# tsnorri/vcf2multialign

Hardware: AMD Instinct MI355X
Metric: aligned A2M Gbases/sec (higher is better)
Workload: dtype u8

## Files before the change

### vcf2multialign_amd/csrc/kernels.hpp

```cpp
#pragma once

#include <hip/hip_runtime.h>
#include <stdint.h>

#ifdef V2M_CHECKED_BUILD
__device__ uint32_t v2m_lds_poison_seed;
#endif

namespace v2m {

typedef uint32_t u32;
typedef uint64_t u64;

constexpr int kWave = 64;
typedef u32 vec4u __attribute__((ext_vector_type(4)));
typedef vec4u vec4u_unaligned8 __attribute__((aligned(8)));

#ifdef V2M_CHECKED_BUILD
__device__ __forceinline__ u32 poison_hash(u32 seed, u32 wg, u32 i)
{
	u32 h = seed ^ (wg * 0x9E3779B1u) ^ (i * 0x85EBCA77u);
	h ^= h >> 15; h *= 0x2C1B3C6Du;
	h ^= h >> 12; h *= 0x297A2D39u;
	h ^= h >> 15;
// ... 1413 lines not shown
{
	splice_aligned_tiles<kNonTemporal, true, true>(tmpl, eff, eff_words_per_row, tt, patches, labels, out, row_pitch, n_rows, rows_per_group, n_groups,
		n_tiles, tile_run, 0, gap, 0u, 0u, st);
}


__device__ __forceinline__ u32 zero_bytes_mask(u32 x)
{
	return ~(((x & 0x7F7F7F7Fu) + 0x7F7F7F7Fu) | x | 0x7F7F7F7Fu);
}

__device__ __forceinline__ u32 wave_inclusive_scan_u32(u32 v)
{
	v += (u32) __builtin_amdgcn_update_dpp(0, (int) v, 0x111, 0xf, 0xf, false);
	v += (u32) __builtin_amdgcn_update_dpp(0, (int) v, 0x112, 0xf, 0xf, false);
	v += (u32) __builtin_amdgcn_update_dpp(0, (int) v, 0x114, 0xf, 0xf, false);
	v += (u32) __builtin_amdgcn_update_dpp(0, (int) v, 0x118, 0xf, 0xf, false);
	v += (u32) __builtin_amdgcn_update_dpp(0, (int) v, 0x142, 0xa, 0xf, false);
	v += (u32) __builtin_amdgcn_update_dpp(0, (int) v, 0x143, 0xc, 0xf, false);
	return v;
}

template <int kN>
__device__ __forceinline__ void wave_inclusive_scan_u32_lockstep(u32 (&v)[kN])
{
#define V2M_SCAN_ROUND(CTRL, ROWS) \
	_Pragma("unroll") for (int k = 0; k < kN; ++k) v[k] += (u32) __builtin_amdgcn_update_dpp(0, (int) v[k], CTRL, ROWS, 0xf, false);
	V2M_SCAN_ROUND(0x111, 0xf)
	V2M_SCAN_ROUND(0x112, 0xf)
	V2M_SCAN_ROUND(0x114, 0xf)
	V2M_SCAN_ROUND(0x118, 0xf)
	V2M_SCAN_ROUND(0x142, 0xa)
	V2M_SCAN_ROUND(0x143, 0xc)
#undef V2M_SCAN_ROUND
}

__device__ __forceinline__ u64 wave_shift_left_u64(u64 v)
{
	u32 const lo = (u32) __builtin_amdgcn_update_dpp(0, (int) (u32) v, 0x130, 0xf, 0xf, true);
	u32 const hi = (u32) __builtin_amdgcn_update_dpp(0, (int) (u32) (v >> 32), 0x130, 0xf, 0xf, true);
	return (u64) hi << 32 | lo;
}

__device__ __forceinline__ u32 count_nonzero_bytes(unsigned char const *tile, u32 lo, u32 hi)
{
	u32 n = 0;
	while (lo < hi && (lo & 3)) n += tile[lo++] != 0;
	for (; lo + 4 <= hi; lo += 4)
		n += 4 - __builtin_popcount(zero_bytes_mask(*(u32 const *) (tile + lo)));
	while (lo < hi) n += tile[lo++] != 0;
	return n;
}

constexpr int kCountRowsMax = 256;
constexpr int kCandDeltaLds = 1024;

template <bool kWindow, bool kSet = false>
__device__ __forceinline__ void count_unaligned_tiles(
	vec4u const *__restrict__ tmpl0, u64 const *__restrict__ eff, u64 eff_words_per_row,
	tile_tables tt, edge_patch const *__restrict__ patches, char const *__restrict__ labels,
	u32 *__restrict__ tile_counts , u32 n_tiles,
	u32 n_rows, u32 rows_per_group, u32 n_groups, u32 tile_run, u32 col_base, u32 col_end, set_tile_tables const st = set_tile_tables{})
{
	__shared__ vec4u lds[kTileChunks];
	__shared__ patch_cache pc;
	__shared__ int row_delta[kCountRowsMax];
	__shared__ int cand_delta[kCandDeltaLds];
	__shared__ u32 wave_sums[kSpliceThreads / 64];

	int const t = threadIdx.x;
	u32 tile, group;
	map_block(blockIdx.x, n_groups, n_tiles, tile_run, tile, group);
	u32 const row_begin = group * rows_per_group;
	u32 const row_end = (row_begin + rows_per_group < n_rows) ? row_begin + rows_per_group : n_rows;
	V2M_POISON_LDS(lds);
	V2M_POISON_LDS(pc);
	V2M_POISON_LDS(row_delta);
	V2M_POISON_LDS(cand_delta);
	V2M_POISON_LDS(wave_sums);

	u32 const n_chunks = kSet ? set_tile_chunks(st, tile) : (u32) kTileChunks;
	u32 mine = 0;
#pragma unroll
	for (int k = 0; k < kChunksPerThread; ++k) {
		if (kSet && (u32) (t + kSpliceThreads * k) >= n_chunks) continue;
		vec4u const v = tmpl0[(kSet ? (u64) (st.record_offset[tile] >> 4) : (u64) tile * kTileChunks) + t + kSpliceThreads * k];
		lds[t + kSpliceThreads * k] = v;
#pragma unroll
		for (int d = 0; d < 4; ++d)
			mine += 4 - __builtin_popcount(zero_bytes_mask(v[d]));
	}
#pragma unroll
	for (int d = 32; d >= 1; d >>= 1) mine += __shfl_down(mine, d, kWave);
	if ((t & 63) == 0) wave_sums[t >> 6] = mine;
	for (u32 r = t; r < (u32) kCountRowsMax; r += kSpliceThreads) row_delta[r] = 0;

	tile_job job;
	load_patch_cache<kWindow, kSet>(pc, job, tt, patches, labels, eff, eff_words_per_row, tile, row_begin, row_end - row_begin, t, col_base, col_end, st);
	__syncthreads();
	u32 tile_count = 0;
#pragma unroll
	for (int wv = 0; wv < kSpliceThreads / 64; ++wv) tile_count += wave_sums[wv];

	unsigned char const *const tile_bytes = (unsigned char const *) lds;
	auto patch_delta = [&](tile_patch const &tp) {
		u32 const label_end = tp.aln_begin + tp.label_len;
		int const label_in_tile = label_end > tp.from ? (int) ((label_end < tp.to ? label_end : tp.to) - tp.from) : 0;
		return label_in_tile - (int) count_nonzero_bytes(tile_bytes, tp.from - job.tile_base, tp.to - job.tile_base);
	};
	u32 const n_cand = job.n_cross + job.n_range;
	for (u32 i = t; i < n_cand && i < (u32) kCandDeltaLds; i += kSpliceThreads)
		cand_delta[i] = patch_delta(candidate_patch<kWindow>(pc, job, patches, i, candidate_edge(job, tt, i), candidate_in_lds(job, i)));
	__syncthreads();
	for (u32 sub = row_begin; sub < row_end; sub += kGroupRowsLds) {
		u32 const sub_end = sub + kGroupRowsLds < row_end ? sub + kGroupRowsLds : row_end;
		if (sub != row_begin) {
			asm volatile("s_waitcnt lgkmcnt(0)" ::: "memory");
			__syncthreads();
			load_eff_cache(pc, job, eff, eff_words_per_row, sub, sub_end - sub, t);
			__syncthreads();
		}
		u32 const sub_rows = sub_end - sub;
		u32 const nw = job.n_lds ? ((job.range_begin + job.n_lds - 1) >> 6) - job.w0 + 1 : 0;
		for (u32 idx = t; idx < sub_rows * nw; idx += kSpliceThreads) {
			u32 const r = idx / nw, w = idx % nw;
			u32 const first = (job.w0 + w) * 64u;
			u64 bits = pc.eff[r][w];
			if (first < job.range_begin) bits &= ~0ULL << (job.range_begin - first);
			u32 const cached_end = job.range_begin + job.n_lds;
			if (cached_end < first + 64u) bits &= (1ULL << (cached_end - first)) - 1;
			int delta = 0;
			for (; bits; bits &= bits - 1) {
				u32 const e = first + (u32) __builtin_ctzll(bits);
				u32 const i = job.n_cross + (e - job.range_begin);
				delta += i < (u32) kCandDeltaLds ? cand_delta[i] : patch_delta(candidate_patch<kWindow>(pc, job, patches, i, e, true));
			}
			if (delta) atomicAdd(&row_delta[sub - row_begin + r], delta);
		}
		u32 const n_other = n_cand - job.n_lds;
		for (u32 idx = t; idx < sub_rows * n_other; idx += kSpliceThreads) {
			u32 const r = idx / n_other, j = idx % n_other;
			u32 const i = j < job.n_cross ? j : j + job.n_lds;
			u32 const e = candidate_edge(job, tt, i);
			if (!((eff[(u64) (sub + r) * eff_words_per_row + (e >> 6)] >> (e & 63)) & 1)) continue;
			int const delta = i < (u32) kCandDeltaLds ? cand_delta[i] : patch_delta(candidate_patch<kWindow>(pc, job, patches, i, e, false));
			if (delta) atomicAdd(&row_delta[sub - row_begin + r], delta);
		}
	}
	__syncthreads();
	for (u32 r = t; r < row_end - row_begin; r += kSpliceThreads)
		tile_counts[(u64) (row_begin + r) * n_tiles + tile] = (u32) ((int) tile_count + row_delta[r]);
}

__global__ __launch_bounds__(kSpliceThreads) void count_unaligned_kernel(
	vec4u const *__restrict__ tmpl0, u64 const *__restrict__ eff, u64 eff_words_per_row,
	tile_tables tt, edge_patch const *__restrict__ patches, char const *__restrict__ labels,
	u32 *__restrict__ tile_counts , u32 n_tiles,
	u32 n_rows, u32 rows_per_group, u32 n_groups, u32 tile_run)
{
	count_unaligned_tiles<false>(tmpl0, eff, eff_words_per_row, tt, patches, labels, tile_counts, n_tiles, n_rows, rows_per_group, n_groups, tile_run, 0u, 0u);
}

__global__ __launch_bounds__(kSpliceThreads) void count_unaligned_window_kernel(
	vec4u const *__restrict__ tmpl0, u64 const *__restrict__ eff, u64 eff_words_per_row,
	tile_tables tt, edge_patch const *__restrict__ patches, char const *__restrict__ labels,
	u32 *__restrict__ tile_counts , u32 n_tiles,
	u32 n_rows, u32 rows_per_group, u32 n_groups, u32 tile_run, u32 col_base, u32 col_end)
{
	count_unaligned_tiles<true>(tmpl0, eff, eff_words_per_row, tt, patches, labels, tile_counts, n_tiles, n_rows, rows_per_group, n_groups, tile_run, col_base, col_end);
}

__global__ __launch_bounds__(kSpliceThreads) void count_unaligned_set_kernel(
	vec4u const *__restrict__ tmpl0, u64 const *__restrict__ eff, u64 eff_words_per_row,
	tile_tables tt, set_tile_tables st, edge_patch const *__restrict__ patches, char const *__restrict__ labels,
	u32 *__restrict__ tile_counts , u32 n_tiles,
	u32 n_rows, u32 rows_per_group, u32 n_groups, u32 tile_run)
{
	count_unaligned_tiles<true, true>(tmpl0, eff, eff_words_per_row, tt, patches, labels, tile_counts, n_tiles, n_rows, rows_per_group, n_groups, tile_run, 0u, 0u, st);
}

__device__ __forceinline__ u32 compaction_selector(u32 keep)
{
	u32 sel = 0x0c0c0c0cu, n = 0;
	for (u32 b = 0; b < 4; ++b)
		if (keep >> b & 1) { sel = (sel & ~(0xFFu << (8 * n))) | (b << (8 * n)); ++n; }
	return sel;
}

typedef unsigned short u16;
typedef u16 u16_unaligned __attribute__((aligned(1)));
typedef u32 u32_unaligned __attribute__((aligned(1)));
typedef u64 u64_unaligned __attribute__((aligned(1)));
typedef vec4u vec4u_unaligned __attribute__((aligned(1)));

#ifdef V2M_TUNING_BUILD
template <bool kNonTemporal>
__global__ __launch_bounds__(kSpliceThreads) void splice_unaligned_per_wave_kernel(
	vec4u const *__restrict__ tmpl0, u64 const *__restrict__ eff, u64 eff_words_per_row,
	tile_tables tt, edge_patch const *__restrict__ patches, char const *__restrict__ labels,
	u32 const *__restrict__ tile_offsets , u32 n_tiles,
	char *__restrict__ out, u64 row_pitch, u32 n_rows, u32 rows_per_group, u32 n_groups, u32 tile_run)
{
	__shared__ vec4u lds[kTileChunks];
	__shared__ patch_cache pc;
	__shared__ u32 wave_sums[kChunksPerThread * (kSpliceThreads / 64)];
	__shared__ u32 compact_sel[16];
	constexpr u32 kPackQueue = 24;
	__shared__ u32 pack_queue[kSpliceThreads / 64][kPackQueue];

	int const t = threadIdx.x;
	int const lane = t & 63, wave = __builtin_amdgcn_readfirstlane(t >> 6);
	if (t < 16) compact_sel[t] = compaction_selector((u32) t);
	u32 tile, group;
	map_block(blockIdx.x, n_groups, n_tiles, tile_run, tile, group);
	{
		u32 const t0 = tile / tile_run * tile_run;
		u32 const run = (n_tiles - t0 < tile_run) ? n_tiles - t0 : tile_run;
		if (0 == run % 8) { u32 const j = tile - t0; tile = t0 + (j & 7) * (run / 8) + (j >> 3); }
	}
	u32 const row_begin = group * rows_per_group;
	u32 const row_end = (row_begin + rows_per_group < n_rows) ? row_begin + rows_per_group : n_rows;

	vec4u pristine[kChunksPerThread];
#pragma unroll
	for (int k = 0; k < kChunksPerThread; ++k)
		pristine[k] = tmpl0[(u64) tile * kTileChunks + t + kSpliceThreads * k];

	tile_job job;
	load_patch_cache(pc, job, tt, patches, labels, eff, eff_words_per_row, tile, row_begin, row_end - row_begin, t);

	for (u32 row = row_begin; row < row_end; ++row) {
// ... 1115 lines not shown
```

### vcf2multialign_amd/csrc/v2m_hip.hip

```cpp

#include <hip/hip_runtime.h>

#include <algorithm>
#include <atomic>
#include <chrono>
#include <condition_variable>
#include <cstdarg>
#include <cstdio>
#include <cstdlib>
#include <cstring>
#include <functional>
#include <memory>
#include <mutex>
#include <string>
#include <thread>
#include <utility>
#include <vector>

#include <type_traits>
#include <unordered_map>

#include "../../include/v2m_hip.h"
#include "kernels.hpp"
#include "founder_kernels.hpp"
// ... 80 lines not shown
		hipError_t const st(dev_buf::ensure(n));
#ifdef V2M_CHECKED_BUILD
		if (hipSuccess == st && !fresh) return poison_device(p, bytes);
#else
		(void) fresh;
#endif
		return st;
	}
};

struct pinned_buf {
	void *p{};
	size_t bytes{};
	~pinned_buf() { reset(); }
	void reset() { if (p) (void) hipHostFree(p); p = nullptr; bytes = 0; }
	hipError_t ensure(size_t n)
	{
		if (n <= bytes) return hipSuccess;
		reset();
		if (0 == n) return hipSuccess;
		hipError_t const st(hipHostMalloc(&p, n, hipHostMallocDefault));
		if (hipSuccess == st) bytes = n; else p = nullptr;
		return st;
	}
	template <typename T> T *as() const { return static_cast<T *>(p); }
};

struct event_pair { hipEvent_t begin{}, end{}; };

}


struct held_ring_state {
	std::mutex mutex;
	std::condition_variable released;
};

struct v2m_row_hold {
	pinned_buf host;
	hipEvent_t copied{};
	uint64_t outstanding{};
	held_ring_state *ring{};
};


struct word_range { u64 restart, lo, hi, stride; };

struct row_view {
	u64 begin{}, end{};
	u64 max_unaligned{};
	u32 n_tiles{};
	dev_buf d_template, d_template0;
	bool has_template0{};
	dev_buf d_edge_begin, d_cross_offsets, d_cross_edges;
	word_range words{};
	u64 length() const { return end - begin; }
};


struct v2m_ctx {
	int device{};
	u32 n_cus{256};
	hipStream_t stream{};
	hipStream_t copy_stream{};
	std::string err;

	bool profiling{};
	std::vector<event_pair> events[V2M_KERNEL_LIMIT];
	std::vector<event_pair> free_events;

	bool has_graph{};
	u64 n_nodes{}, n_edges{}, ref_len{}, aligned_len{}, label_bytes{};
	bool has_nul_byte{};
	std::vector<u32> h_csum;
	std::vector<u32> h_tgt_prefix_max;
	dev_buf d_ref, d_ref_pos, d_aln_pos, d_spans, d_patches, d_labels, d_overlappable;
	dev_buf d_ovl_rank, d_blocker_masks;
	std::vector<u32> h_aln_pos, h_tile_edge_begin, h_cross_offsets, h_cross_edges;
	std::vector<v2m::edge_patch> h_patches;
	std::vector<u64> h_overlappable;

	row_view whole, window;
	bool windowed{};
	row_view &view() { return set_call ? set.view : windowed ? window : whole; }
	row_view const &view() const { return set_call ? set.view : windowed ? window : whole; }

	struct window_set {
		row_view view;
		u64 n_windows{}, pitch{}, mean_tile_bytes{};
		std::vector<u32> lengths;
		dev_buf d_col_begin, d_col_end, d_record_offset, d_edge_end, d_tile_window, d_first_tile, d_slot_offset32;
	} set;
	bool has_set{}, set_call{};
	scratch_buf d_set_tile_offsets, d_set_lengths[2];
	int set_lengths_slot{};
	scratch_buf d_distinct_keys, d_distinct_windows, d_distinct_items, d_distinct_flags;
	pinned_buf h_distinct_keys, h_distinct_items, h_distinct_flags;

	u64 const *d_paths{};
	dev_buf owned_paths;
	dev_buf d_slice_src;
	u64 path_rows{}, path_cols{};
	u64 path_pitch{};
	dev_buf d_by_edge;
	bool by_edge_valid{};

// ... 696 lines not shown
		launch(0 != mode);
	}
	V2M_HIP_TRY(ctx, hipGetLastError());
	return V2M_OK;
}


v2m::set_tile_tables set_tables(v2m_ctx const *ctx)
{
	auto const &s(ctx->set);
	return {s.d_col_begin.as<u32>(), s.d_col_end.as<u32>(), s.d_record_offset.as<u32>(), s.d_edge_end.as<u32>()};
}

int expand_reference_set(v2m_ctx *ctx, dev_buf &dst, char gap);


int splice_aligned_slice(v2m_ctx *ctx, v2m_row_batch const *rows, u64 row_begin, u64 row_end, char *d_out, u64 row_pitch)
{
	u64 const n_rows(row_end - row_begin);
	if (0 == n_rows || 0 == ctx->aligned_len) return V2M_OK;
	if (int const rc = resolve_slice(ctx, rows, row_begin, row_end)) return rc;

	row_view const &v(ctx->view());
	splice_grid g;
	if (int const rc = make_grid(ctx, n_rows, g)) return rc;
	v2m::tile_tables const tt{v.d_edge_begin.as<u32>(), v.d_cross_offsets.as<u32>(), v.d_cross_edges.as<u32>()};
	u64 const store_limit((v.length() + 15) & ~u64(15));
	auto const launch([&](bool nt) {
		auto const go([&](auto kernel, auto... window) {
			hipLaunchKernelGGL(kernel, dim3(unsigned(g.n_blocks)), dim3(v2m::kSpliceThreads), 0, ctx->stream,
				v.d_template.as<v2m::vec4u>(), ctx->d_eff.as<u64>() - v.words.restart, v.words.stride, tt, ctx->d_patches.as<v2m::edge_patch>(), ctx->d_labels.as<char>(),
				d_out, row_pitch, u32(n_rows), g.rows_per_group, g.n_groups, v.n_tiles, g.tile_run, store_limit, '-', window...);
		});
		if (ctx->set_call) {
			auto const go_set([&](auto kernel) {
				hipLaunchKernelGGL(kernel, dim3(unsigned(g.n_blocks)), dim3(v2m::kSpliceThreads), 0, ctx->stream,
					v.d_template.as<v2m::vec4u>(), ctx->d_eff.as<u64>() - v.words.restart, v.words.stride, tt, set_tables(ctx), ctx->d_patches.as<v2m::edge_patch>(), ctx->d_labels.as<char>(),
					d_out, row_pitch, u32(n_rows), g.rows_per_group, g.n_groups, v.n_tiles, g.tile_run, '-');
			});
			if (nt) go_set(v2m::splice_aligned_set_kernel<true>);
			else go_set(v2m::splice_aligned_set_kernel<false>);
		}
		else if (ctx->windowed) {
			if (nt) go(v2m::splice_aligned_window_kernel<true>, u32(v.begin), u32(v.end));
			else go(v2m::splice_aligned_window_kernel<false>, u32(v.begin), u32(v.end));
		}
		else if (nt) go(v2m::splice_aligned_kernel<true>);
		else go(v2m::splice_aligned_kernel<false>);
	});
	return store_flavour_launch(ctx, false, n_rows, n_rows * v.length(), launch);
}


int splice_unaligned_slice(v2m_ctx *ctx, v2m_row_batch const *rows, u64 row_begin, u64 row_end, char *d_out, u64 row_pitch)
{
	u64 const n_rows(row_end - row_begin);
	if (0 == n_rows) return V2M_OK;
	V2M_HIP_TRY(ctx, ctx->d_row_lengths.ensure(n_rows * sizeof(u64)));
	if (0 == ctx->aligned_len) {
		V2M_HIP_TRY(ctx, hipMemsetAsync(ctx->d_row_lengths.p, 0, n_rows * sizeof(u64), ctx->stream));
		return V2M_OK;
	}
	row_view &v(ctx->view());
	bool const set(ctx->set_call);
	if (!v.has_template0) {
		if (int const rc = set ? expand_reference_set(ctx, v.d_template0, 0) : expand_reference(ctx, v, v.d_template0, 0)) return rc;
		v.has_template0 = true;
	}
	if (int const rc = resolve_slice(ctx, rows, row_begin, row_end)) return rc;

	splice_grid g;
	if (int const rc = make_grid(ctx, n_rows, g)) return rc;
	V2M_HIP_TRY(ctx, ctx->d_tile_counts.ensure(n_rows * v.n_tiles * sizeof(u32)));
	if (set) {
		V2M_HIP_TRY(ctx, ctx->d_set_tile_offsets.ensure(n_rows * v.n_tiles * sizeof(u32)));
		V2M_HIP_TRY(ctx, ctx->d_set_lengths[ctx->set_lengths_slot].ensure(n_rows * ctx->set.n_windows * sizeof(u32)));
	}
	bool const windowed(ctx->windowed);
	v2m::tile_tables const tt{v.d_edge_begin.as<u32>(), v.d_cross_offsets.as<u32>(), v.d_cross_edges.as<u32>()};
	u64 const *const d_eff(ctx->d_eff.as<u64>() - v.words.restart);
	{
		char const *const ce(std::getenv("V2M_COUNT_ROWS_PER_GROUP"));
		u32 const count_rows(u32(std::min<u64>(std::max<u64>(1, n_rows), (ce && *ce && std::atoi(ce) > 0) ? u64(std::min(std::atoi(ce), int(v2m::kCountRowsMax))) : u64(v2m::kCountRowsMax))));
		u32 const count_groups(u32((n_rows + count_rows - 1) / count_rows));
		timed_launch tl(ctx, V2M_KERNEL_UNALIGNED_COUNT);
		auto const count([&](auto kernel, auto... window) {
			hipLaunchKernelGGL(kernel, dim3(unsigned(u64(v.n_tiles) * count_groups)), dim3(v2m::kSpliceThreads), 0, ctx->stream,
				v.d_template0.as<v2m::vec4u>(), d_eff, v.words.stride, tt, ctx->d_patches.as<v2m::edge_patch>(), ctx->d_labels.as<char>(),
				ctx->d_tile_counts.as<u32>(), v.n_tiles, u32(n_rows), count_rows, count_groups, g.tile_run, window...);
		});
		if (set)
			hipLaunchKernelGGL(v2m::count_unaligned_set_kernel, dim3(unsigned(u64(v.n_tiles) * count_groups)), dim3(v2m::kSpliceThreads), 0, ctx->stream,
				v.d_template0.as<v2m::vec4u>(), d_eff, v.words.stride, tt, set_tables(ctx), ctx->d_patches.as<v2m::edge_patch>(), ctx->d_labels.as<char>(),
				ctx->d_tile_counts.as<u32>(), v.n_tiles, u32(n_rows), count_rows, count_groups, g.tile_run);
		else if (windowed) count(v2m::count_unaligned_window_kernel, u32(v.begin), u32(v.end));
		else count(v2m::count_unaligned_kernel);
		hipLaunchKernelGGL(v2m::scan_tile_counts_kernel, dim3(unsigned(n_rows)), dim3(256), 0, ctx->stream,
			ctx->d_tile_counts.as<u32>(), v.n_tiles, ctx->d_row_lengths.as<u64>());
		if (set)
			hipLaunchKernelGGL(v2m::scan_window_set_kernel, dim3(unsigned(n_rows)), dim3(256), 0, ctx->stream,
				ctx->d_tile_counts.as<u32>(), ctx->d_row_lengths.as<u64>(), v.n_tiles, u32(ctx->set.n_windows),
				ctx->set.d_first_tile.as<u32>(), ctx->set.d_tile_window.as<u32>(), ctx->set.d_slot_offset32.as<u32>(),
				ctx->d_set_tile_offsets.as<u32>(), ctx->d_set_lengths[ctx->set_lengths_slot].as<u32>());
	}
	auto const launch([&](bool nt) {
		auto const go([&](auto kernel, auto... window) {
			hipLaunchKernelGGL(kernel, dim3(unsigned(g.n_blocks)), dim3(v2m::kSpliceThreads), 0, ctx->stream,
				v.d_template0.as<v2m::vec4u>(), d_eff, v.words.stride, tt, ctx->d_patches.as<v2m::edge_patch>(), ctx->d_labels.as<char>(),
				ctx->d_tile_counts.as<u32>(), v.n_tiles, d_out, row_pitch, u32(n_rows), g.rows_per_group, g.n_groups, g.tile_run, window...);
		});
		if (set) {
			auto const go_set([&](auto kernel) {
				hipLaunchKernelGGL(kernel, dim3(unsigned(g.n_blocks)), dim3(v2m::kSpliceThreads), 0, ctx->stream,
					v.d_template0.as<v2m::vec4u>(), d_eff, v.words.stride, tt, set_tables(ctx), ctx->d_patches.as<v2m::edge_patch>(), ctx->d_labels.as<char>(),
					ctx->d_set_tile_offsets.as<u32>(), v.n_tiles, d_out, row_pitch, u32(n_rows), g.rows_per_group, g.n_groups, g.tile_run);
			});
			if (nt) go_set(v2m::splice_unaligned_set_kernel<true>);
			else go_set(v2m::splice_unaligned_set_kernel<false>);
			return;
		}
		if (windowed) {
			if (nt) go(v2m::splice_unaligned_window_kernel<true>, u32(v.begin), u32(v.end));
			else go(v2m::splice_unaligned_window_kernel<false>, u32(v.begin), u32(v.end));
			return;
		}
#ifdef V2M_TUNING_BUILD
		static int const flavour([] { char const *const e(std::getenv("V2M_UNALIGNED_KERNEL")); return !e ? 0 : 0 == std::strcmp(e, "wave") ? 1 : 0 == std::strcmp(e, "shared64") ? 2 : 0; }());
		if (1 == flavour) { if (nt) go(v2m::splice_unaligned_per_wave_kernel<true>); else go(v2m::splice_unaligned_per_wave_kernel<false>); return; }
		if (2 == flavour) { if (nt) go(v2m::splice_unaligned_kernel<true, 64>); else go(v2m::splice_unaligned_kernel<false, 64>); return; }
#endif
		if (nt) go(v2m::splice_unaligned_kernel<true>);
		else go(v2m::splice_unaligned_kernel<false>);
	});
	return store_flavour_launch(ctx, true, n_rows, n_rows * ((set || windowed) ? v.length() : ctx->ref_len), launch);
// ... 597 lines not shown
			blocker_masks.push_back(mask);
		}
	}
	ovl_rank.back() = u32(blocker_masks.size());

	u32 const n_tiles(u32(std::max<u64>(1, (L + v2m::kTileBytes - 1) / v2m::kTileBytes)));
	std::vector<u32> tile_edge_begin(n_tiles + 1), cross_offsets(n_tiles + 1, 0), cross_edges;
	{
		u32 e(0);
		for (u32 t(0); t <= n_tiles; ++t) {
			u64 const base(u64(t) * v2m::kTileBytes);
			while (e < E && patches[e].aln_begin < base) ++e;
			tile_edge_begin[t] = e;
		}
		tile_edge_begin[n_tiles] = u32(E);
		std::vector<u32> counts(n_tiles + 1, 0);
		auto for_each_crossing = [&](auto &&fn) {
			for (u32 e2(0); e2 < E; ++e2) {
				u64 const first(u64(patches[e2].aln_begin) / v2m::kTileBytes + 1);
				if (0 == patches[e2].aln_end) continue;
				u64 const last((u64(patches[e2].aln_end) - 1) / v2m::kTileBytes);
				for (u64 t(first); t <= last && t < n_tiles; ++t) fn(u32(t), e2);
			}
		};
		for_each_crossing([&](u32 t, u32) { ++counts[t]; });
		for (u32 t(0); t < n_tiles; ++t) cross_offsets[t + 1] = cross_offsets[t] + counts[t];
		cross_edges.resize(cross_offsets[n_tiles]);
		std::vector<u32> cursor(cross_offsets.begin(), cross_offsets.end() - 1);
		for_each_crossing([&](u32 t, u32 e2) { cross_edges[cursor[t]++] = e2; });
	}

	ctx->has_graph = false;
	ctx->windowed = false;
	ctx->has_set = false;
	ctx->n_nodes = N; ctx->n_edges = E; ctx->ref_len = ref_len; ctx->aligned_len = L; ctx->label_bytes = label_total;
	V2M_HIP_TRY(ctx, ctx->d_ref.ensure(std::max<u64>(ref_len, 16)));
	if (ref_len) V2M_HIP_TRY(ctx, hipMemcpyAsync(ctx->d_ref.p, ref_seq, ref_len, hipMemcpyHostToDevice, ctx->stream));
	V2M_HIP_TRY(ctx, ctx->d_labels.ensure(std::max<u64>(label_total, 16)));
	if (label_total) V2M_HIP_TRY(ctx, hipMemcpyAsync(ctx->d_labels.p, g->alt_edge_label_bytes, label_total, hipMemcpyHostToDevice, ctx->stream));
	if (int const rc = upload_vec(ctx, ctx->d_ref_pos, ref_pos)) return rc;
	if (int const rc = upload_vec(ctx, ctx->d_aln_pos, aln_pos)) return rc;
	if (int const rc = upload_vec(ctx, ctx->d_spans, spans)) return rc;
	if (int const rc = upload_vec(ctx, ctx->d_patches, patches)) return rc;
	if (int const rc = upload_vec(ctx, ctx->d_overlappable, overlappable)) return rc;
	if (int const rc = upload_vec(ctx, ctx->d_ovl_rank, ovl_rank)) return rc;
	if (int const rc = upload_vec(ctx, ctx->d_blocker_masks, blocker_masks)) return rc;

	row_view &v(ctx->whole);
	v.begin = 0;
	v.end = L;
	v.max_unaligned = ref_len + label_total;
	v.n_tiles = n_tiles;
	v.has_template0 = false;
	ctx->has_ops_ref_before = false;
	v.words = {0, 0, (E + 63) / 64, (((E + 63) / 64) + 15) & ~u64(15)};
	if (int const rc = upload_vec(ctx, v.d_edge_begin, tile_edge_begin)) return rc;
	if (int const rc = upload_vec(ctx, v.d_cross_offsets, cross_offsets)) return rc;
	if (int const rc = upload_vec(ctx, v.d_cross_edges, cross_edges)) return rc;
	if (int const rc = expand_reference(ctx, v, v.d_template, '-')) return rc;

	ctx->d_paths = nullptr;
	ctx->by_edge_valid = false;
	ctx->path_rows = ctx->path_cols = ctx->path_pitch = 0;
	if (g->paths_by_chrom_copy_and_edge) {
		size_t const bytes(g->path_rows / 64 * g->path_cols * sizeof(u64));
		V2M_HIP_TRY(ctx, ctx->owned_paths.ensure(std::max<size_t>(bytes, 16)));
		if (bytes) V2M_HIP_TRY(ctx, hipMemcpyAsync(ctx->owned_paths.p, g->paths_by_chrom_copy_and_edge, bytes, hipMemcpyHostToDevice, ctx->stream));
		ctx->d_paths = ctx->owned_paths.as<u64>();
		ctx->path_rows = g->path_rows;
		ctx->path_cols = g->path_cols;
		ctx->path_pitch = g->path_rows / 64;
	}
	V2M_HIP_TRY(ctx, hipStreamSynchronize(ctx->stream));

	ctx->has_nul_byte = (ref_len && std::memchr(ref_seq, 0, ref_len)) || (label_total && std::memchr(g->alt_edge_label_bytes, 0, label_total));
	ctx->h_csum = std::move(csum);
	ctx->h_tgt_prefix_max = std::move(tgt_prefix_max);
	ctx->h_aln_pos = std::move(aln_pos);
	ctx->h_patches = std::move(patches);
	ctx->h_overlappable = std::move(overlappable);
	ctx->h_tile_edge_begin = std::move(tile_edge_begin);
	ctx->h_cross_offsets = std::move(cross_offsets);
	ctx->h_cross_edges = std::move(cross_edges);
	ctx->has_graph = true;
	return V2M_OK;
}

int v2m_set_paths_device(v2m_ctx *ctx, const void *d_words, uint64_t path_rows, uint64_t path_cols)
{
	if (!ctx) return V2M_ERR_INVALID_ARGUMENT;
	if (!ctx->has_graph) return fail(ctx, V2M_ERR_STATE, "no graph uploaded");
	if (path_rows % 64 || path_cols % 64 || path_rows < ctx->n_edges)
		return fail(ctx, V2M_ERR_PRECONDITION, "path matrix must be (>= edge_count) x copies with both dimensions multiples of 64");
	if (path_rows && path_cols && (!d_words || ((uintptr_t) d_words & 7))) return fail(ctx, V2M_ERR_INVALID_ARGUMENT, "d_words must be a non-NULL 8-byte aligned device pointer");
	ctx->d_paths = static_cast<u64 const *>(d_words);
	ctx->by_edge_valid = false;
	ctx->path_rows = path_rows;
	ctx->path_cols = path_cols;
	ctx->path_pitch = path_rows / 64;
	return V2M_OK;
}

namespace {

u64 aligned_pitch(u64 words) { return (words + 15) & ~u64(15); }

// ... 144 lines not shown
		tb.cross_offsets.push_back(u32(tb.cross_edges.size()));
		begin = end;
	}
}

u64 first_edge_reaching_past(v2m_ctx const *ctx, u64 col_begin, u32 e_hi)
{
	u64 e_lo(0), hi(e_hi);
	while (e_lo < hi) {
		u64 const mid((e_lo + hi) / 2);
		if (ctx->h_aln_pos[ctx->h_tgt_prefix_max[mid + 1]] > col_begin) hi = mid; else e_lo = mid + 1;
	}
	return e_lo;
}

word_range words_of_edges(v2m_ctx const *ctx, u64 e_lo, u64 e_hi)
{
	u64 restart(0), lo(0), word_hi(0);
	if (e_lo < e_hi) {
		lo = e_lo / 64;
		word_hi = (e_hi + 63) / 64;
		restart = lo;
		while (restart > 0 && (ctx->h_overlappable[restart] & 1)) --restart;
	}
	return {restart, lo, word_hi, (word_hi - restart + 15) & ~u64(15)};
}

}


int v2m_set_column_window(v2m_ctx *ctx, uint64_t col_begin, uint64_t col_end)
{
	if (!ctx) return V2M_ERR_INVALID_ARGUMENT;
	if (!ctx->has_graph) return fail(ctx, V2M_ERR_STATE, "no graph uploaded");
	u64 const L(ctx->aligned_len);
	if (!(col_begin < col_end && col_end <= L))
		return fail(ctx, V2M_ERR_INVALID_ARGUMENT, "column window [%llu, %llu) is empty or not within the aligned length %llu",
			(unsigned long long) col_begin, (unsigned long long) col_end, (unsigned long long) L);
	ctx->windowed = false;
	if (0 == col_begin && L == col_end) return V2M_OK;
	V2M_HIP_TRY(ctx, hipSetDevice(ctx->device));

	window_tile_tables tb;
	append_window_tiles(ctx, col_begin, col_end, tb);
	u32 const e_hi(tb.edge_end.back());
	tb.edge_begin.push_back(e_hi);
	row_view &w(ctx->window);
	w.words = words_of_edges(ctx, first_edge_reaching_past(ctx, col_begin, e_hi), e_hi);
	w.begin = col_begin;
	w.end = col_end;
	w.max_unaligned = col_end - col_begin;
	w.n_tiles = u32(tb.edge_end.size());
	w.has_template0 = false;
	if (int const rc = upload_vec(ctx, w.d_edge_begin, tb.edge_begin)) return rc;
	if (int const rc = upload_vec(ctx, w.d_cross_offsets, tb.cross_offsets)) return rc;
	if (int const rc = upload_vec(ctx, w.d_cross_edges, tb.cross_edges)) return rc;
	if (int const rc = expand_reference(ctx, w, w.d_template, '-')) return rc;
	V2M_HIP_TRY(ctx, hipStreamSynchronize(ctx->stream));
	ctx->windowed = true;
	return V2M_OK;
}



int v2m_window_set_layout(uint64_t n_windows, const uint64_t *col_begin, const uint64_t *col_end, uint64_t *slot_offset, uint64_t *record_pitch)
{
	if (0 == n_windows) return fail(nullptr, V2M_ERR_INVALID_ARGUMENT, "a window set needs at least one window");
	if (!col_begin || !col_end) return fail(nullptr, V2M_ERR_INVALID_ARGUMENT, "NULL array");
	u64 at(0);
	for (u64 k(0); k < n_windows; ++k) {
		if (!(col_begin[k] < col_end[k]))
			return fail(nullptr, V2M_ERR_INVALID_ARGUMENT, "window %llu, [%llu, %llu), is empty", (unsigned long long) k, (unsigned long long) col_begin[k], (unsigned long long) col_end[k]);
		if (slot_offset) slot_offset[k] = at;
		u64 const len(col_end[k] - col_begin[k]);
		if (len >= (u64(1) << 32) || (at += (len + 15) & ~u64(15)) >= (u64(1) << 32))
			return fail(nullptr, V2M_ERR_UNSUPPORTED, "the slots of the window set reach 2^32 bytes at window %llu: split the set", (unsigned long long) k);
	}
	if (record_pitch) *record_pitch = (at + 255) & ~u64(255);
	return V2M_OK;
}

uint64_t v2m_window_set_size(const v2m_ctx *ctx) { return (ctx && ctx->has_graph && ctx->has_set) ? ctx->set.n_windows : 0; }
uint64_t v2m_window_set_pitch(const v2m_ctx *ctx) { return (ctx && ctx->has_graph && ctx->has_set) ? ctx->set.pitch : 0; }

namespace {

int expand_reference_set(v2m_ctx *ctx, dev_buf &dst, char gap)
{
	u64 const n_chunks(ctx->set.view.end / 16);
	V2M_HIP_TRY(ctx, dst.ensure(n_chunks * 16));
	{
		timed_launch tl(ctx, V2M_KERNEL_TEMPLATE);
		hipLaunchKernelGGL(v2m::expand_reference_set_kernel, dim3(unsigned((n_chunks + 255) / 256)), dim3(256), 0, ctx->stream,
			ctx->d_ref.as<char>(), ctx->d_ref_pos.as<u32>(), ctx->d_aln_pos.as<u32>(), u32(ctx->n_nodes), set_tables(ctx), ctx->set.view.n_tiles, n_chunks, dst.as<uint4>(), gap);
	}
	V2M_HIP_TRY(ctx, hipGetLastError());
	return V2M_OK;
}

struct scoped_set_call {
	v2m_ctx *ctx;
	explicit scoped_set_call(v2m_ctx *c) : ctx(c) { c->set_call = true; }
	~scoped_set_call() { ctx->set_call = false; }
};

int check_set_call(v2m_ctx *ctx, v2m_row_batch const *rows, u32 flags)
// ... 10 lines not shown
{
	if (!ctx) return V2M_ERR_INVALID_ARGUMENT;
	if (!ctx->has_graph) return fail(ctx, V2M_ERR_STATE, "no graph uploaded");
	if (0 == n_windows) return fail(ctx, V2M_ERR_INVALID_ARGUMENT, "a window set needs at least one window");
	if (!col_begin || !col_end) return fail(ctx, V2M_ERR_INVALID_ARGUMENT, "NULL array");
	u64 const L(ctx->aligned_len);
	u64 n_tiles(0);
	for (u64 k(0); k < n_windows; ++k) {
		if (!(col_begin[k] < col_end[k] && col_end[k] <= L))
			return fail(ctx, V2M_ERR_INVALID_ARGUMENT, "window %llu, [%llu, %llu), is empty or not within the aligned length %llu",
				(unsigned long long) k, (unsigned long long) col_begin[k], (unsigned long long) col_end[k], (unsigned long long) L);
		n_tiles += (col_end[k] - col_begin[k] + v2m::kTileBytes - 1) / v2m::kTileBytes;
	}
	std::vector<u64> slot_offset(n_windows);
	u64 pitch(0);
	if (int const rc = v2m_window_set_layout(n_windows, col_begin, col_end, slot_offset.data(), &pitch)) return fail(ctx, rc, "%s", g_create_error.c_str());
	if (n_windows >= 0xFFFFFFFFull || n_tiles >= 0x7FFFFFFFull)
		return fail(ctx, V2M_ERR_UNSUPPORTED, "the window set has too many tiles (%llu) for one set: split it", (unsigned long long) n_tiles);
	ctx->has_set = false;
	V2M_HIP_TRY(ctx, hipSetDevice(ctx->device));

	auto &set(ctx->set);
	window_tile_tables tb;
	std::vector<u32> tile_col_begin, tile_col_end, tile_record_offset, tile_window, first_tile(n_windows + 1), slot_offset32(n_windows);
	tile_col_begin.reserve(n_tiles); tile_col_end.reserve(n_tiles); tile_record_offset.reserve(n_tiles); tile_window.reserve(n_tiles);
	set.lengths.resize(n_windows);
	u64 e_lo(~u64(0)), e_hi(0), slots_end(0);
	for (u64 k(0); k < n_windows; ++k) {
		u64 const len(col_end[k] - col_begin[k]);
		first_tile[k] = tb.n_tiles();
		slot_offset32[k] = u32(slot_offset[k]);
		set.lengths[k] = u32(len);
		slots_end = slot_offset[k] + ((len + 15) & ~u64(15));
		append_window_tiles(ctx, col_begin[k], col_end[k], tb);
		for (u64 j(0); j * v2m::kTileBytes < len; ++j) {
			tile_col_begin.push_back(u32(col_begin[k] + j * v2m::kTileBytes));
			tile_col_end.push_back(u32(std::min<u64>(col_begin[k] + (j + 1) * v2m::kTileBytes, col_end[k])));
			tile_record_offset.push_back(u32(slot_offset[k] + j * v2m::kTileBytes));
			tile_window.push_back(u32(k));
		}
		u32 const w_hi(tb.edge_end.back());
		u64 const w_lo(first_edge_reaching_past(ctx, col_begin[k], w_hi));
		if (w_lo < w_hi) { e_lo = std::min(e_lo, w_lo); e_hi = std::max<u64>(e_hi, w_hi); }
	}
	first_tile[n_windows] = tb.n_tiles();
	tb.edge_begin.push_back(0);
	row_view &v(set.view);
	v.words = words_of_edges(ctx, std::min(e_lo, e_hi), e_hi);
	v.begin = 0;
	v.end = slots_end;
	v.max_unaligned = slots_end;
	v.n_tiles = tb.n_tiles();
	v.has_template0 = false;
	set.n_windows = n_windows;
	set.pitch = pitch;
	u64 total(0);
	for (u32 const len : set.lengths) total += len;
	set.mean_tile_bytes = std::max<u64>(1, total / v.n_tiles);
	if (int const rc = upload_vec(ctx, v.d_edge_begin, tb.edge_begin)) return rc;
	if (int const rc = upload_vec(ctx, v.d_cross_offsets, tb.cross_offsets)) return rc;
	if (int const rc = upload_vec(ctx, v.d_cross_edges, tb.cross_edges)) return rc;
	if (int const rc = upload_vec(ctx, set.d_edge_end, tb.edge_end)) return rc;
	if (int const rc = upload_vec(ctx, set.d_col_begin, tile_col_begin)) return rc;
	if (int const rc = upload_vec(ctx, set.d_col_end, tile_col_end)) return rc;
	if (int const rc = upload_vec(ctx, set.d_record_offset, tile_record_offset)) return rc;
	if (int const rc = upload_vec(ctx, set.d_tile_window, tile_window)) return rc;
	if (int const rc = upload_vec(ctx, set.d_first_tile, first_tile)) return rc;
	if (int const rc = upload_vec(ctx, set.d_slot_offset32, slot_offset32)) return rc;
	if (int const rc = expand_reference_set(ctx, v.d_template, '-')) return rc;
	V2M_HIP_TRY(ctx, hipStreamSynchronize(ctx->stream));
	ctx->has_set = true;
	return V2M_OK;
}

int v2m_splice_window_set(v2m_ctx *ctx, const v2m_row_batch *rows, uint32_t flags, v2m_window_sink_fn sink, void *user)
{
	if (int const rc = check_set_call(ctx, rows, flags)) return rc;
	if (!sink) return fail(ctx, V2M_ERR_INVALID_ARGUMENT, "sink is NULL");
	if (0 == rows->n_rows) return V2M_OK;
	V2M_HIP_TRY(ctx, hipSetDevice(ctx->device));
	scoped_set_call const in_set(ctx);
	u64 const n_windows(ctx->set.n_windows);
	return splice_rows_pipeline(ctx, rows, flags & V2M_SPLICE_UNALIGNED, 2, "v2m_splice_window_set", [&](v2m_row_hold &, slot_rows const &sl) -> int {
		for (u64 r(sl.r0); r < sl.r1; ++r)
			if (sink(user, r, sl.row(r), sl.set_lengths ? sl.set_lengths + (r - sl.r0) * n_windows : ctx->set.lengths.data()))
				return fail(ctx, V2M_ERR_SINK, "sink aborted at row %llu", (unsigned long long) r);
		return V2M_OK;
	});
}

int v2m_splice_window_set_device(v2m_ctx *ctx, const v2m_row_batch *rows, uint32_t flags, void *d_out, uint64_t record_pitch, uint32_t *lengths_out)
{
	if (int const rc = check_set_call(ctx, rows, flags)) return rc;
	if (0 == rows->n_rows) return V2M_OK;
	if (!d_out || ((uintptr_t) d_out & 15)) return fail(ctx, V2M_ERR_INVALID_ARGUMENT, "d_out must be a 16-byte aligned device pointer");
	if (record_pitch % 16 || record_pitch < ctx->set.view.end)
		return fail(ctx, V2M_ERR_INVALID_ARGUMENT, "record_pitch must be a multiple of 16 and at least the end of the last slot, %llu", (unsigned long long) ctx->set.view.end);
	V2M_HIP_TRY(ctx, hipSetDevice(ctx->device));
	scoped_set_call const in_set(ctx);
	u64 const n_windows(ctx->set.n_windows);
	if (!(flags & V2M_SPLICE_UNALIGNED)) {
		if (int const rc = splice_aligned_slice(ctx, rows, 0, rows->n_rows, static_cast<char *>(d_out), record_pitch)) return rc;
		if (lengths_out)
			for (u64 r(0); r < rows->n_rows; ++r) std::copy(ctx->set.lengths.begin(), ctx->set.lengths.end(), lengths_out + r * n_windows);
		return V2M_OK;
	}
// ... 565 lines not shown
	V2M_HIP_TRY(ctx, hipSetDevice(ctx->device));
	auto &state(ctx->held_state);
	return splice_rows_pipeline(ctx, rows, flags & V2M_SPLICE_UNALIGNED, n_slots, "v2m_splice_rows_held", [&](v2m_row_hold &slot, slot_rows const &sl) -> int {
		{ std::lock_guard<std::mutex> const lock(state.mutex); slot.outstanding = sl.r1 - sl.r0; }
		for (u64 r(sl.r0); r < sl.r1; ++r) {
			if (0 == sink(user, r, sl.row(r), sl.bytes(r), &slot)) continue;
			{ std::lock_guard<std::mutex> const lock(state.mutex); slot.outstanding -= sl.r1 - r; }
			return fail(ctx, V2M_ERR_SINK, "sink aborted at row %llu", (unsigned long long) r);
		}
		return V2M_OK;
	});
}

void v2m_row_release(v2m_row_hold *hold)
{
	if (!hold) return;
	std::lock_guard<std::mutex> const lock(hold->ring->mutex);
	if (hold->outstanding && 0 == --hold->outstanding) hold->ring->released.notify_all();
}




namespace {

struct scoped_whole_rows {
	v2m_ctx *ctx;
	bool was;
	explicit scoped_whole_rows(v2m_ctx *c) : ctx(c), was(c->windowed) { c->windowed = false; }
	~scoped_whole_rows() { ctx->windowed = was; }
};

u64 ops_slice_budget()
{
	char const *const e(std::getenv("V2M_OPS_SLICE_BYTES"));
	return (e && *e) ? std::strtoull(e, nullptr, 10) : (u64(64) << 20);
}

int row_ops_count_slice(v2m_ctx *ctx, v2m_row_batch const *rows, u64 row_begin, u64 row_end, bool split, u64 *total_ops)
{
	u64 const n_rows(row_end - row_begin);
	row_view &v(ctx->whole);
	if (int const rc = resolve_slice(ctx, rows, row_begin, row_end)) return rc;
	splice_grid g;
	if (int const rc = make_grid(ctx, n_rows, g)) return rc;
	u64 const cells(n_rows * v.n_tiles);
	V2M_HIP_TRY(ctx, ctx->d_row_lengths.ensure(n_rows * sizeof(u64)));
	V2M_HIP_TRY(ctx, ctx->d_tile_counts.ensure(cells * sizeof(u32)));
	V2M_HIP_TRY(ctx, ctx->d_ops_info.ensure(cells * sizeof(u32)));
	V2M_HIP_TRY(ctx, ctx->d_ops_offsets.ensure(cells * sizeof(u32)));
	V2M_HIP_TRY(ctx, ctx->d_ops_counts.ensure(n_rows * sizeof(u32)));
	v2m::tile_tables const tt{v.d_edge_begin.as<u32>(), v.d_cross_offsets.as<u32>(), v.d_cross_edges.as<u32>()};
	u64 const *const d_eff(ctx->d_eff.as<u64>() - v.words.restart);
	{
		u32 const count_rows(u32(std::min<u64>(n_rows, u64(v2m::kCountRowsMax))));
		u32 const count_groups(u32((n_rows + count_rows - 1) / count_rows));
		timed_launch tl(ctx, V2M_KERNEL_UNALIGNED_COUNT);
		hipLaunchKernelGGL(v2m::count_unaligned_kernel, dim3(unsigned(u64(v.n_tiles) * count_groups)), dim3(v2m::kSpliceThreads), 0, ctx->stream,
			v.d_template0.as<v2m::vec4u>(), d_eff, v.words.stride, tt, ctx->d_patches.as<v2m::edge_patch>(), ctx->d_labels.as<char>(),
			ctx->d_tile_counts.as<u32>(), v.n_tiles, u32(n_rows), count_rows, count_groups, g.tile_run);
		hipLaunchKernelGGL(v2m::scan_tile_counts_kernel, dim3(unsigned(n_rows)), dim3(256), 0, ctx->stream,
			ctx->d_tile_counts.as<u32>(), v.n_tiles, ctx->d_row_lengths.as<u64>());
	}
	{
		timed_launch tl(ctx, V2M_KERNEL_ROW_OPS_COUNT);
		hipLaunchKernelGGL(split ? v2m::count_row_ops_eqx_kernel : v2m::count_row_ops_kernel, dim3(unsigned(g.n_blocks)), dim3(v2m::kSpliceThreads), 0, ctx->stream,
			v.d_template0.as<v2m::vec4u>(), d_eff, v.words.stride, tt, ctx->d_patches.as<v2m::edge_patch>(), ctx->d_labels.as<char>(),
			ctx->d_ops_info.as<u32>(), v.n_tiles, u32(n_rows), g.rows_per_group, g.n_groups, g.tile_run);
	}
	{
		timed_launch tl(ctx, V2M_KERNEL_ROW_OPS_SCAN);
		hipLaunchKernelGGL(split ? v2m::scan_row_ops_eqx_kernel : v2m::scan_row_ops_kernel, dim3(unsigned(n_rows)), dim3(256), 0, ctx->stream,
			ctx->d_ops_info.as<u32>(), ctx->d_ops_offsets.as<u32>(), v.n_tiles, ctx->d_ops_counts.as<u32>());
	}
	V2M_HIP_TRY(ctx, hipGetLastError());
	u64 const counts_bytes((n_rows * sizeof(u32) + 7) & ~u64(7));
	V2M_HIP_TRY(ctx, ctx->h_ops_stage.ensure(counts_bytes + 2 * n_rows * sizeof(u64)));
	V2M_POISON_HOST(ctx->h_ops_stage.p, counts_bytes + 2 * n_rows * sizeof(u64));
	char *const stage(ctx->h_ops_stage.as<char>());
	V2M_HIP_TRY(ctx, hipMemcpyAsync(stage, ctx->d_ops_counts.p, n_rows * sizeof(u32), hipMemcpyDeviceToHost, ctx->stream));
	V2M_HIP_TRY(ctx, hipMemcpyAsync(stage + counts_bytes, ctx->d_row_lengths.p, n_rows * sizeof(u64), hipMemcpyDeviceToHost, ctx->stream));
	V2M_HIP_TRY(ctx, hipStreamSynchronize(ctx->stream));
	u32 const *const counts(reinterpret_cast<u32 const *>(stage));
	*total_ops = 0;
	for (u64 r(0); r < n_rows; ++r) *total_ops += counts[r];
	return V2M_OK;
}

int row_ops_emit_piece(v2m_ctx *ctx, u64 slice_begin, u64 slice_rows, u64 piece_begin, u64 piece_end, bool split, v2m_ops_sink_fn sink, void *user)
{
	u64 const n_rows(piece_end - piece_begin);
	row_view &v(ctx->whole);
	u64 const counts_bytes((slice_rows * sizeof(u32) + 7) & ~u64(7));
	char *const stage(ctx->h_ops_stage.as<char>());
	u32 const *const counts(reinterpret_cast<u32 const *>(stage) + piece_begin);
	u64 const *const lengths(reinterpret_cast<u64 const *>(stage + counts_bytes) + piece_begin);
	u64 *const bases(reinterpret_cast<u64 *>(stage + counts_bytes + slice_rows * sizeof(u64)) + piece_begin);
	u64 total_ops(0);
	for (u64 r(0); r < n_rows; ++r) { bases[r] = total_ops; total_ops += counts[r]; }
	v2m::row_op_record const *records(nullptr);
	if (total_ops) {
		splice_grid g;
		if (int const rc = make_grid(ctx, n_rows, g)) return rc;
		V2M_HIP_TRY(ctx, ctx->d_ops_base.ensure(n_rows * sizeof(u64)));
		V2M_HIP_TRY(ctx, ctx->d_ops_out.ensure(total_ops * sizeof(v2m::row_op_record)));
		V2M_HIP_TRY(ctx, ctx->h_ops_out.ensure(total_ops * sizeof(v2m::row_op_record)));
		V2M_POISON_HOST(ctx->h_ops_out.p, total_ops * sizeof(v2m::row_op_record));
// ... 2111 lines not shown
```

Before: 6889.

## Precompute per-edge count deltas and fuse per-row count with tile scan

Adds a one-time kernel that computes, for every tile, its base nonzero-byte count and a short delta for each edge patch (begin and cross), cached per row view. A new per-row streaming kernel then sums the deltas of the row's active edges from the effective bitmask and performs the prefix scan over tiles in the same pass. This replaces the per-(tile,row-group) kernel that reloaded template tiles into LDS and recounted bytes, and also drops the separate scan launch. It is on by default for non-set, non-windowed paths and can be turned off with V2M_COUNT_KERNEL=tiles. The cost is extra global memory for the delta tables, and one block per row that loops serially over tiles, which may expose latency when there are many tiles and few rows.

```diff
diff --git a/vcf2multialign_amd/csrc/kernels.hpp b/vcf2multialign_amd/csrc/kernels.hpp
--- a/vcf2multialign_amd/csrc/kernels.hpp
+++ b/vcf2multialign_amd/csrc/kernels.hpp
@@ -1489,6 +1489,13 @@
 	return n;
 }
 
+__device__ __forceinline__ int tile_patch_delta(unsigned char const *tile_bytes, u32 tile_base, tile_patch const &tp)
+{
+	u32 const label_end = tp.aln_begin + tp.label_len;
+	int const label_in_tile = label_end > tp.from ? (int) ((label_end < tp.to ? label_end : tp.to) - tp.from) : 0;
+	return label_in_tile - (int) count_nonzero_bytes(tile_bytes, tp.from - tile_base, tp.to - tile_base);
+}
+
 constexpr int kCountRowsMax = 256;
 constexpr int kCandDeltaLds = 1024;
 
@@ -1540,11 +1547,7 @@
 	for (int wv = 0; wv < kSpliceThreads / 64; ++wv) tile_count += wave_sums[wv];
 
 	unsigned char const *const tile_bytes = (unsigned char const *) lds;
-	auto patch_delta = [&](tile_patch const &tp) {
-		u32 const label_end = tp.aln_begin + tp.label_len;
-		int const label_in_tile = label_end > tp.from ? (int) ((label_end < tp.to ? label_end : tp.to) - tp.from) : 0;
-		return label_in_tile - (int) count_nonzero_bytes(tile_bytes, tp.from - job.tile_base, tp.to - job.tile_base);
-	};
+	auto patch_delta = [&](tile_patch const &tp) { return tile_patch_delta(tile_bytes, job.tile_base, tp); };
 	u32 const n_cand = job.n_cross + job.n_range;
 	for (u32 i = t; i < n_cand && i < (u32) kCandDeltaLds; i += kSpliceThreads)
 		cand_delta[i] = patch_delta(candidate_patch<kWindow>(pc, job, patches, i, candidate_edge(job, tt, i), candidate_in_lds(job, i)));
@@ -1614,6 +1617,132 @@
 	u32 n_rows, u32 rows_per_group, u32 n_groups, u32 tile_run)
 {
 	count_unaligned_tiles<true, true>(tmpl0, eff, eff_words_per_row, tt, patches, labels, tile_counts, n_tiles, n_rows, rows_per_group, n_groups, tile_run, 0u, 0u, st);
+}
+
+typedef short count_delta;
+static_assert(kTileBytes <= 32767, "count_delta holds a tile's bytes either way");
+
+__global__ __launch_bounds__(kSpliceThreads) void build_count_tables_kernel(
+	vec4u const *__restrict__ tmpl0, tile_tables tt, edge_patch const *__restrict__ patches, char const *__restrict__ labels,
+	u32 *__restrict__ tile_base , count_delta *__restrict__ delta_begin , count_delta *__restrict__ delta_cross )
+{
+	__shared__ vec4u lds[kTileChunks];
+	__shared__ patch_cache pc;
+	__shared__ u32 wave_sums[kSpliceThreads / 64];
+
+	int const t = threadIdx.x;
+	u32 const tile = blockIdx.x;
+	V2M_POISON_LDS(lds);
+	V2M_POISON_LDS(pc);
+	V2M_POISON_LDS(wave_sums);
+
+	u32 mine = 0;
+#pragma unroll
+	for (int k = 0; k < kChunksPerThread; ++k) {
+		vec4u const v = tmpl0[(u64) tile * kTileChunks + t + kSpliceThreads * k];
+		lds[t + kSpliceThreads * k] = v;
+#pragma unroll
+		for (int d = 0; d < 4; ++d)
+			mine += 4 - __builtin_popcount(zero_bytes_mask(v[d]));
+	}
+#pragma unroll
+	for (int d = 32; d >= 1; d >>= 1) mine += __shfl_down(mine, d, kWave);
+	if ((t & 63) == 0) wave_sums[t >> 6] = mine;
+
+	tile_job job;
+	load_patch_cache<false>(pc, job, tt, patches, labels, nullptr, 0, tile, 0, 0, t);
+	__syncthreads();
+	if (0 == t) {
+		u32 tile_count = 0;
+#pragma unroll
+		for (int wv = 0; wv < kSpliceThreads / 64; ++wv) tile_count += wave_sums[wv];
+		tile_base[tile] = tile_count;
+	}
+
+	unsigned char const *const tile_bytes = (unsigned char const *) lds;
+	u32 const n_cand = job.n_cross + job.n_range;
+	for (u32 i = t; i < n_cand; i += kSpliceThreads) {
+		int const delta = tile_patch_delta(tile_bytes, job.tile_base, candidate_patch<false>(pc, job, patches, i, candidate_edge(job, tt, i), candidate_in_lds(job, i)));
+		if (i < job.n_cross) delta_cross[job.cross_begin + i] = (count_delta) delta;
+		else delta_begin[job.range_begin + (i - job.n_cross)] = (count_delta) delta;
+	}
+}
+
+constexpr int kCountStreamThreads = 1024;
+
+__global__ __launch_bounds__(kCountStreamThreads) void count_scan_stream_kernel(
+	u64 const *__restrict__ eff, u64 eff_words_per_row, tile_tables tt,
+	u32 const *__restrict__ tile_base, count_delta const *__restrict__ delta_begin, count_delta const *__restrict__ delta_cross,
+	u32 *__restrict__ tile_offsets , u32 n_tiles, u64 *__restrict__ row_lengths)
+{
+	__shared__ u32 wave_sums[2][kCountStreamThreads / 64];
+	V2M_POISON_LDS(wave_sums);
+	int const t = threadIdx.x, lane = t & 63, wave = t >> 6;
+	u64 const *const eff_row = eff + (u64) blockIdx.x * eff_words_per_row;
+	u32 *const row = tile_offsets + (u64) blockIdx.x * n_tiles;
+	u32 carry = 0;
+	struct tile_entry { u32 base, e0, e1, k0, k1; };
+	if (0 == n_tiles) {
+		if (t == 0) row_lengths[blockIdx.x] = 0;
+		return;
+	}
+	auto const load_entry = [&](u32 tile) {
+		u32 const c = tile < n_tiles ? tile : n_tiles - 1;
+		return tile_entry{tile_base[c], tt.edge_begin[c], tt.edge_begin[c + 1], tt.cross_offsets[c], tt.cross_offsets[c + 1]};
+	};
+	tile_entry next = load_entry(t);
+	for (u32 base = 0, trip = 0; base < n_tiles; base += kCountStreamThreads, ++trip) {
+		u32 const tile = base + t;
+		tile_entry const cur = next;
+		next = load_entry(tile + kCountStreamThreads);
+		u32 mine = 0;
+		if (tile < n_tiles) {
+			int count = (int) cur.base;
+			u32 const e0 = cur.e0, e1 = cur.e1;
+			if (e0 < e1) {
+				u32 const w_last = (e1 - 1) >> 6;
+				u64 next_word = eff_row[e0 >> 6];
+				for (u32 w = e0 >> 6; w <= w_last; ++w) {
+					u32 const first = w * 64u;
+					u64 bits = next_word;
+					if (w < w_last) next_word = eff_row[w + 1];
+					if (first < e0) bits &= ~0ULL << (e0 - first);
+					if (e1 - first < 64u) bits &= (1ULL << (e1 - first)) - 1;
+					while (bits) {
+						int d[4];
+#pragma unroll
+						for (int j = 0; j < 4; ++j) {
+							bool const has = bits != 0;
+							d[j] = delta_begin[has ? first + (u32) __builtin_ctzll(bits) : e0];
+							if (!has) d[j] = 0;
+							bits &= bits - 1;
+						}
+						count += d[0] + d[1] + d[2] + d[3];
+					}
+				}
+			}
+			for (u32 k = cur.k0, k_end = cur.k1; k < k_end; ++k) {
+				u32 const e = tt.cross_edges[k];
+				if ((eff_row[e >> 6] >> (e & 63)) & 1) count += delta_cross[k];
+			}
+			mine = (u32) count;
+		}
+		u32 const incl = wave_inclusive_scan_u32(mine);
+		u32 *const sums = wave_sums[trip & 1];
+		if (lane == 63) sums[wave] = incl;
+		asm volatile("s_waitcnt lgkmcnt(0)" ::: "memory");
+		__syncthreads();
+		u32 before = carry, total = 0;
+#pragma unroll
+		for (int wv = 0; wv < kCountStreamThreads / 64; ++wv) {
+			u32 const ws = sums[wv];
+			if (wv < wave) before += ws;
+			total += ws;
+		}
+		if (tile < n_tiles) row[tile] = before + incl - mine;
+		carry += total;
+	}
+	if (t == 0) row_lengths[blockIdx.x] = carry;
 }
 
 __device__ __forceinline__ u32 compaction_selector(u32 keep)
diff --git a/vcf2multialign_amd/csrc/v2m_hip.hip b/vcf2multialign_amd/csrc/v2m_hip.hip
--- a/vcf2multialign_amd/csrc/v2m_hip.hip
+++ b/vcf2multialign_amd/csrc/v2m_hip.hip
@@ -156,6 +156,8 @@
 	u32 n_tiles{};
 	dev_buf d_template, d_template0;
 	bool has_template0{};
+	dev_buf d_count_base, d_delta_begin, d_delta_cross;
+	bool has_count_tables{};
 	dev_buf d_edge_begin, d_cross_offsets, d_cross_edges;
 	word_range words{};
 	u64 length() const { return end - begin; }
@@ -958,6 +960,49 @@
 }
 
 
+bool count_kernel_streams()
+{
+	char const *const e(std::getenv("V2M_COUNT_KERNEL"));
+	return !(e && 0 == std::strcmp(e, "tiles"));
+}
+
+int ensure_count_tables(v2m_ctx *ctx)
+{
+	row_view &v(ctx->whole);
+	if (v.has_count_tables) return V2M_OK;
+	u64 const n_cross(ctx->h_cross_offsets.empty() ? 0 : ctx->h_cross_offsets.back());
+	V2M_HIP_TRY(ctx, v.d_count_base.ensure(std::max<size_t>(v.n_tiles * sizeof(u32), 16)));
+	V2M_HIP_TRY(ctx, v.d_delta_begin.ensure(std::max<size_t>(ctx->n_edges * sizeof(v2m::count_delta), 16)));
+	V2M_HIP_TRY(ctx, v.d_delta_cross.ensure(std::max<size_t>(n_cross * sizeof(v2m::count_delta), 16)));
+	v2m::tile_tables const tt{v.d_edge_begin.as<u32>(), v.d_cross_offsets.as<u32>(), v.d_cross_edges.as<u32>()};
+	{
+		timed_launch tl(ctx, V2M_KERNEL_TEMPLATE);
+		hipLaunchKernelGGL(v2m::build_count_tables_kernel, dim3(v.n_tiles), dim3(v2m::kSpliceThreads), 0, ctx->stream,
+			v.d_template0.as<v2m::vec4u>(), tt, ctx->d_patches.as<v2m::edge_patch>(), ctx->d_labels.as<char>(),
+			v.d_count_base.as<u32>(), v.d_delta_begin.as<v2m::count_delta>(), v.d_delta_cross.as<v2m::count_delta>());
+	}
+	V2M_HIP_TRY(ctx, hipGetLastError());
+	v.has_count_tables = true;
+	return V2M_OK;
+}
+
+int count_scan_stream(v2m_ctx *ctx, u64 n_rows)
+{
+	if (int const rc = ensure_count_tables(ctx)) return rc;
+	row_view &v(ctx->whole);
+	v2m::tile_tables const tt{v.d_edge_begin.as<u32>(), v.d_cross_offsets.as<u32>(), v.d_cross_edges.as<u32>()};
+	{
+		timed_launch tl(ctx, V2M_KERNEL_UNALIGNED_COUNT);
+		hipLaunchKernelGGL(v2m::count_scan_stream_kernel, dim3(unsigned(n_rows)), dim3(v2m::kCountStreamThreads), 0, ctx->stream,
+			ctx->d_eff.as<u64>() - v.words.restart, v.words.stride, tt,
+			v.d_count_base.as<u32>(), v.d_delta_begin.as<v2m::count_delta>(), v.d_delta_cross.as<v2m::count_delta>(),
+			ctx->d_tile_counts.as<u32>(), v.n_tiles, ctx->d_row_lengths.as<u64>());
+	}
+	V2M_HIP_TRY(ctx, hipGetLastError());
+	return V2M_OK;
+}
+
+
 int splice_unaligned_slice(v2m_ctx *ctx, v2m_row_batch const *rows, u64 row_begin, u64 row_end, char *d_out, u64 row_pitch)
 {
 	u64 const n_rows(row_end - row_begin);
@@ -985,7 +1030,10 @@
 	bool const windowed(ctx->windowed);
 	v2m::tile_tables const tt{v.d_edge_begin.as<u32>(), v.d_cross_offsets.as<u32>(), v.d_cross_edges.as<u32>()};
 	u64 const *const d_eff(ctx->d_eff.as<u64>() - v.words.restart);
-	{
+	if (!set && !windowed && count_kernel_streams()) {
+		if (int const rc = count_scan_stream(ctx, n_rows)) return rc;
+	}
+	else {
 		char const *const ce(std::getenv("V2M_COUNT_ROWS_PER_GROUP"));
 		u32 const count_rows(u32(std::min<u64>(std::max<u64>(1, n_rows), (ce && *ce && std::atoi(ce) > 0) ? u64(std::min(std::atoi(ce), int(v2m::kCountRowsMax))) : u64(v2m::kCountRowsMax))));
 		u32 const count_groups(u32((n_rows + count_rows - 1) / count_rows));
@@ -1689,6 +1737,7 @@
 	v.max_unaligned = ref_len + label_total;
 	v.n_tiles = n_tiles;
 	v.has_template0 = false;
+	v.has_count_tables = false;
 	ctx->has_ops_ref_before = false;
 	v.words = {0, 0, (E + 63) / 64, (((E + 63) / 64) + 15) & ~u64(15)};
 	if (int const rc = upload_vec(ctx, v.d_edge_begin, tile_edge_begin)) return rc;
@@ -1939,6 +1988,7 @@
 	w.max_unaligned = col_end - col_begin;
 	w.n_tiles = u32(tb.edge_end.size());
 	w.has_template0 = false;
+	w.has_count_tables = false;
 	if (int const rc = upload_vec(ctx, w.d_edge_begin, tb.edge_begin)) return rc;
 	if (int const rc = upload_vec(ctx, w.d_cross_offsets, tb.cross_offsets)) return rc;
 	if (int const rc = upload_vec(ctx, w.d_cross_edges, tb.cross_edges)) return rc;
@@ -2055,6 +2105,7 @@
 	v.max_unaligned = slots_end;
 	v.n_tiles = tb.n_tiles();
 	v.has_template0 = false;
+	v.has_count_tables = false;
 	set.n_windows = n_windows;
 	set.pitch = pitch;
 	u64 total(0);
@@ -2726,7 +2777,10 @@
 	V2M_HIP_TRY(ctx, ctx->d_ops_counts.ensure(n_rows * sizeof(u32)));
 	v2m::tile_tables const tt{v.d_edge_begin.as<u32>(), v.d_cross_offsets.as<u32>(), v.d_cross_edges.as<u32>()};
 	u64 const *const d_eff(ctx->d_eff.as<u64>() - v.words.restart);
-	{
+	if (count_kernel_streams()) {
+		if (int const rc = count_scan_stream(ctx, n_rows)) return rc;
+	}
+	else {
 		u32 const count_rows(u32(std::min<u64>(n_rows, u64(v2m::kCountRowsMax))));
 		u32 const count_groups(u32((n_rows + count_rows - 1) / count_rows));
 		timed_launch tl(ctx, V2M_KERNEL_UNALIGNED_COUNT);
```

Result: no change. 6881 (median of 2 runs) (-0.1%).
